# sczhou/CodeFormer

Hardware: NVIDIA H100
Metric: faces_per_sec_512x512_batch32 (higher is better)
Workload: dtype f32 (split-fp16 operands on tensor cores, fp32 accumulate)

## Files before the change

### codeformer_b200/csrc/conv_tc.cu

```cuda

#include <cuda.h>
#include <cuda_fp16.h>
#include <cuda_runtime.h>
#include <stdint.h>

#include <stdlib.h>

#include <atomic>
#include <mutex>

#include "conv_tc.cuh"

namespace cfb {

__global__ void tc_absmax_kernel(const float* __restrict__ w, int64_t total, unsigned* __restrict__ slot) {
  float m = 0.f;
  for (int64_t i = (int64_t)blockIdx.x * blockDim.x + threadIdx.x; i < total; i += (int64_t)gridDim.x * blockDim.x)
    m = fmaxf(m, fabsf(w[i]));
#pragma unroll
  for (int o = 16; o > 0; o >>= 1) m = fmaxf(m, __shfl_xor_sync(0xffffffffu, m, o));
  if ((threadIdx.x & 31) == 0) atomicMax(slot, __float_as_uint(m));
}

__global__ void tc_split_weights_kernel(const float* __restrict__ w, __half* __restrict__ hi, __half* __restrict__ lo,
// ... 282 lines not shown

__device__ __forceinline__ void wg_mma_64x128(float (&d)[64], uint64_t da, uint64_t db, uint32_t accum) {
  asm volatile(
      "{\n\t.reg .pred p;\n\t"
      "setp.ne.b32 p, %66, 0;\n\t"
      "wgmma.mma_async.sync.aligned.m64n128k16.f32.f16.f16 "
      "{%0, %1, %2, %3, %4, %5, %6, %7, %8, %9, %10, %11, %12, %13, %14, %15, "
      "%16, %17, %18, %19, %20, %21, %22, %23, %24, %25, %26, %27, %28, %29, %30, %31, "
      "%32, %33, %34, %35, %36, %37, %38, %39, %40, %41, %42, %43, %44, %45, %46, %47, "
      "%48, %49, %50, %51, %52, %53, %54, %55, %56, %57, %58, %59, %60, %61, %62, %63}, %64, %65, p, 1, 1, 0, 0;\n\t}"
      : "+f"(d[0]), "+f"(d[1]), "+f"(d[2]), "+f"(d[3]), "+f"(d[4]), "+f"(d[5]), "+f"(d[6]), "+f"(d[7]), "+f"(d[8]),
        "+f"(d[9]), "+f"(d[10]), "+f"(d[11]), "+f"(d[12]), "+f"(d[13]), "+f"(d[14]), "+f"(d[15]), "+f"(d[16]),
        "+f"(d[17]), "+f"(d[18]), "+f"(d[19]), "+f"(d[20]), "+f"(d[21]), "+f"(d[22]), "+f"(d[23]), "+f"(d[24]),
        "+f"(d[25]), "+f"(d[26]), "+f"(d[27]), "+f"(d[28]), "+f"(d[29]), "+f"(d[30]), "+f"(d[31]), "+f"(d[32]),
        "+f"(d[33]), "+f"(d[34]), "+f"(d[35]), "+f"(d[36]), "+f"(d[37]), "+f"(d[38]), "+f"(d[39]), "+f"(d[40]),
        "+f"(d[41]), "+f"(d[42]), "+f"(d[43]), "+f"(d[44]), "+f"(d[45]), "+f"(d[46]), "+f"(d[47]), "+f"(d[48]),
        "+f"(d[49]), "+f"(d[50]), "+f"(d[51]), "+f"(d[52]), "+f"(d[53]), "+f"(d[54]), "+f"(d[55]), "+f"(d[56]),
        "+f"(d[57]), "+f"(d[58]), "+f"(d[59]), "+f"(d[60]), "+f"(d[61]), "+f"(d[62]), "+f"(d[63])
      : "l"(da), "l"(db), "r"(accum)
      : "memory");
}
__device__ __forceinline__ void wg_wait_1() { asm volatile("wgmma.wait_group.sync.aligned 1;" ::: "memory"); }

__device__ __forceinline__ bool wg_any(bool v, uint32_t bar_id = 2) {
  uint32_t r;
  asm volatile(
      "{\n\t.reg .pred p, q;\n\t"
      "setp.ne.u32 p, %1, 0;\n\t"
      "bar.red.or.pred q, %2, 128, p;\n\t"
      "selp.u32 %0, 1, 0, q;\n\t}"
      : "=r"(r)
      : "r"((uint32_t)v), "r"(bar_id)
      : "memory");
  return r != 0;
}

__device__ __forceinline__ float ex2_ftz(float x) { float r; asm("ex2.approx.ftz.f32 %0, %1;" : "=f"(r) : "f"(x)); return r; }
__device__ __forceinline__ float rcp_ftz(float x) { float r; asm("rcp.approx.ftz.f32 %0, %1;" : "=f"(r) : "f"(x)); return r; }
__device__ __forceinline__ uint32_t pack_f16x2(float lo, float hi) {
  uint32_t r;
  asm("cvt.rn.f16x2.f32 %0, %1, %2;" : "=r"(r) : "f"(hi), "f"(lo));
  return r;
}
__device__ __forceinline__ float f16_minus_f32(uint32_t h, float c) {
  return __half2float(__ushort_as_half((unsigned short)h)) - c;
}
// ... 23 lines not shown
    float y[2];
#pragma unroll
    for (int e = 0; e < 2; ++e) {
      float v = __uint_as_float(raw[2 * q + e]);
      if (MODE >= 1) v = fmaf(v, sc[2 * q + e], sh[2 * q + e]);
      if (MODE == 2) v = v * rcp_ftz(1.f + ex2_ftz(v * -1.4426950408889634f));
      y[e] = v;
    }
    amax = fmaxf(amax, fmaxf(fabsf(y[0]), fabsf(y[1])));
    hw[q] = pack_f16x2(y[0], y[1]);
    if constexpr (LO) {
      const float d0 = f16_minus_f32(hw[q] & 0xffffu, y[0]);
      const float d1 = f16_minus_f32(hw[q] >> 16, y[1]);
      lw[q] = pack_f16x2(d0, d1) ^ 0x80008000u;
    }
  }
  hv = make_uint4(hw[0], hw[1], hw[2], hw[3]);
  if constexpr (LO) lv = make_uint4(lw[0], lw[1], lw[2], lw[3]);
}
template <int MODE, int RPP, int NPASS, int PW, int ROWS, bool LO = true>
__device__ __forceinline__ void xf_patch(uint32_t src_base, uint32_t hi_base, uint32_t lo_base, int c0, int j, int rsub,
                                         const float (&sc)[8], const float (&sh)[8], bool border, int y0, int x0, int Hin,
                                         int Win, float& amax) {
#pragma unroll
  for (int it = 0; it < NPASS; it += 2) {
    uint4 a[2], b[2];
    bool act[2];
#pragma unroll
    for (int u = 0; u < 2; ++u) {
      const int r = rsub + (it + u) * RPP;
      act[u] = (it + u < NPASS) && (r < ROWS);
      if (act[u]) {
        const uint32_t row = src_base + (uint32_t)r * 128u;
        const uint32_t sw = (row >> 7) & 7u;
        a[u] = lds128(row + (((uint32_t)c0 ^ sw) << 4));
        b[u] = lds128(row + (((uint32_t)(c0 + 1) ^ sw) << 4));
      }
    }
    __syncwarp();
#pragma unroll
    for (int u = 0; u < 2; ++u) {
      if (act[u]) {
        const int r = rsub + (it + u) * RPP;
        uint4 hv, lv;
        xf_chunk<MODE, LO>(a[u], b[u], sc, sh, hv, lv, amax);
        if (border) {
          const int py = r / PW, px = r - py * PW;
// ... 57 lines not shown
  __half* pl_hi;
  __half* pl_lo;
  float* gn_part;
  int gn_cpg;
#if CFB_TC_STAMPS
  long long* dbg;
#endif
};
#if CFB_TC_STAMPS
#define TC_STAMP(i) do { if (p.dbg != nullptr && blockIdx.x == 0) p.dbg[i] = clock64(); } while (0)
#else
#define TC_STAMP(i) do { } while (0)
#endif

constexpr int XF_SKEW = 128;
constexpr int TC_A_BYTES = 128 * 128;

template <int BN>
struct TcCfg {
  static_assert(BN == 64 || BN == 128, "the wgmma engine runs 64- or 128-wide n-tiles");
  static constexpr bool WIDE = BN == 128;
  static constexpr int MMA_WARPS = WIDE ? 8 : 4;
  static constexpr int EPI_WARPS = WIDE ? 4 : 8;
  static constexpr int THREADS = 32 * (MMA_WARPS + 1 + EPI_WARPS);
  static constexpr int B_BYTES = BN * 128;
  static constexpr int STAGE_BYTES = 2 * TC_A_BYTES + 2 * B_BYTES;
  static constexpr int STAGES = 3;
  static constexpr int SLOT_PITCH = BN + 4;
  static constexpr int SLOT_BYTES = 128 * SLOT_PITCH * 4;
  static constexpr int SLOTS = 1;
  static constexpr int STG_BYTES = WIDE ? 0 : 8 * 4096;
  static constexpr int TAIL_BYTES = SLOT_BYTES + 1024  + 512  + STG_BYTES;
  static constexpr int SMEM_BYTES = STAGES * STAGE_BYTES + TAIL_BYTES;
  static constexpr int H_A_PLANE = 23 * 1024;
  static constexpr int H_A_SLOT = 2 * H_A_PLANE;
  static constexpr int H_A_SLOTS = 2;
  static constexpr int H_B_SLOT = 2 * B_BYTES;
  static constexpr int H_B_SLOTS = WIDE ? 2 : 4;
  static constexpr int H_SMEM_BYTES = H_A_SLOTS * H_A_SLOT + H_B_SLOTS * H_B_SLOT + TAIL_BYTES;
  static constexpr int XF_WARPS = WIDE ? 2 : 4;
  static constexpr int XF_THREADS = THREADS + 32 * XF_WARPS + 32;
  static constexpr int X_A_SLOTS = 2;
  static constexpr int X_A_PLANE2 = H_A_PLANE + XF_SKEW;
  static constexpr int X_B_SLOTS = H_B_SLOTS;
  static constexpr int X_SMEM_BYTES = X_A_SLOTS * H_A_SLOT + X_B_SLOTS * H_B_SLOT + TAIL_BYTES;
};

template <int BN, int CPG, bool HALO, bool XF, bool GEN = false, bool K1 = false, bool CM = false, bool SILU = false,
          bool P1 = false>
__global__ void __launch_bounds__(XF ? TcCfg<BN>::XF_THREADS : TcCfg<BN>::THREADS, 1)
conv_tc_kernel(const __grid_constant__ CUtensorMap tmA_hi, const __grid_constant__ CUtensorMap tmA_lo,
               const __grid_constant__ CUtensorMap tmB_hi, const __grid_constant__ CUtensorMap tmB_lo, const TcParams p) {
  static_assert(!XF || HALO, "the fused operand transform exists for the halo engine only");
  static_assert(!GEN || (XF && CPG == 0), "the generalised addressing exists for the fused-transform engine only");
  static_assert(!K1 || (XF && !GEN && CPG == 0), "K1 = fused transform of a 1x1 conv (patch = tile): its own instantiation");
  using Cfg = TcCfg<BN>;
  constexpr bool WIDE = Cfg::WIDE;
  static_assert(!WIDE || (HALO && !GEN && !K1 && CPG != 2), "128-wide tiles exist for the 3x3 / Upsample halo engine");
  static_assert(!CM || (BN == 64 && HALO && !GEN && !K1), "channel-major tiles exist for the 64-channel 3x3 / Upsample halo convs");
  static_assert(!P1 || (!SILU && !K1 && (GEN || WIDE || CM || !HALO)),
                "the single-pass fp16 variant is built for the generalised, 128-wide, channel-major and per-tap engines");
  constexpr int MMA_WARPS = Cfg::MMA_WARPS, EPI_WARPS = Cfg::EPI_WARPS;
  constexpr int A_SLOTS = XF ? Cfg::X_A_SLOTS : Cfg::H_A_SLOTS;
  constexpr int STAGES = Cfg::STAGES;
// ... 29 lines not shown
      mbar_init(smem_u32(afull + a), XF ? Cfg::XF_WARPS : 1);
      mbar_init(smem_u32(aempty + a), MMA_WARPS);
      mbar_init(smem_u32(araw + a), 1);
    }
    asm volatile("prefetch.tensormap [%0];" ::"l"(&tmA_hi) : "memory");
    asm volatile("prefetch.tensormap [%0];" ::"l"(&tmA_lo) : "memory");
    asm volatile("prefetch.tensormap [%0];" ::"l"(&tmB_hi) : "memory");
    asm volatile("prefetch.tensormap [%0];" ::"l"(&tmB_lo) : "memory");
    for (int s = 0; s < NRING; ++s) { mbar_init(smem_u32(full + s), 1); mbar_init(smem_u32(empty + s), MMA_WARPS); }
    for (int a = 0; a < Cfg::SLOTS; ++a) {
      mbar_init(smem_u32(cfull + a), MMA_WARPS);
      mbar_init(smem_u32(cempty + a), EPI_WARPS);
    }
    asm volatile("fence.mbarrier_init.release.cluster;" ::: "memory");
  }
  __syncthreads();
  pdl_launch_dependents();
  pdl_wait();
  if (threadIdx.x == 0) TC_STAMP(1);

  const int total_tiles = p.m_tiles * p.n_tiles;
  const int nk = p.taps * p.kblocks;

  if (warp == 0) {
    {
      int stage = 0;
      uint32_t phase = 0;
      int aslot = 0;
      uint32_t aphase = 0;
      for (int tile = first_tile; tile < total_tiles; tile += tile_step) {
        const int mt = tile / p.n_tiles, nt = tile - mt * p.n_tiles;
        const int mtl = p.up4 ? (mt >> 2) : mt;
        const int par_y = p.up4 ? ((mt & 3) >> 1) : 0, par_x = p.up4 ? (mt & 1) : 0;
        const int per_img = p.tiles_x * p.tiles_y;
        const int n = mtl / per_img;
        const int rem = mtl - n * per_img;
        const int ty = rem / p.tiles_x, tx = rem - ty * p.tiles_x;
        const int y0 = ty * p.BH * p.stride, x0 = tx * p.BW * p.stride;
        if constexpr (HALO) {
          for (int kb = 0; kb < p.kblocks; ++kb) {
            if constexpr (!XF) {
              mbar_wait<500>(smem_u32(aempty + aslot), aphase ^ 1, aborted); if (aborted) goto teardown;
              if (elect_one()) {
                const uint32_t sa = smem_u32(smem + aslot * Cfg::H_A_SLOT);
                const uint32_t ab = smem_u32(afull + aslot);
                mbar_expect_tx(ab, (uint32_t)((P1 ? 1 : 2) * p.PW * p.PH * 128));
// ... 29 lines not shown
              if (elect_one()) {
                if (tile == first_tile && tap == 0 && kb == 0) TC_STAMP(2);
                const uint32_t sa = smem_u32(smem + stage * STAGE_BYTES);
                const int hh = p.heads > 1 ? n % p.heads : 0, nimg = p.heads > 1 ? n / p.heads : n;
                const int a_img = p.a_img_per_head ? n : nimg;
                const int ac = p.a_c0 + hh * p.a_c_head + kb * 64, bc = p.b_c0 + hh * p.b_c_head + kb * 64;
                const int brow = nt * BN + hh * p.b_r_head;
                const int b3 = p.b_batched ? nimg : btap;
                const uint32_t fb = smem_u32(full + stage);
                const bool drop = p.fault && blockIdx.x == 0 && tile == first_tile && kb == 0 && tap == 0;
                mbar_expect_tx(fb, (uint32_t)(P1 ? TC_A_BYTES + Cfg::B_BYTES : Cfg::STAGE_BYTES));
                tma_load_4d(sa, &tmA_hi, fb, ac, x0 + s - p.pad, y0 + r - p.pad, a_img);
                if constexpr (!P1) tma_load_4d(sa + TC_A_BYTES, &tmA_lo, fb, ac, x0 + s - p.pad, y0 + r - p.pad, a_img);
                if (!drop) tma_load_3d(sa + 2 * TC_A_BYTES, &tmB_hi, fb, bc, brow, b3);
                if constexpr (!P1) tma_load_3d(sa + 2 * TC_A_BYTES + Cfg::B_BYTES, &tmB_lo, fb, bc, brow, b3);
              }
              __syncwarp();
              if (++stage == STAGES) { stage = 0; phase ^= 1; }
            }
          }
        }
      }
    }
  } else if (warp == 1) {
    {
      constexpr bool N128 = WIDE || CM;
      constexpr int MH = N128 ? 1 : 2;
      const uint32_t a_sbo = HALO ? (uint32_t)(p.PW * 128) : 1024u;
      const uint32_t a_half = HALO ? (uint32_t)(8 * p.PW * 128) : 8192u;
      const int wq = (int)(threadIdx.x >> 5) & 3;
      const int wg = (int)(threadIdx.x >> 7);
      const uint32_t bar_id = 2u + (uint32_t)wg;
      const uint32_t slot_base = smem_u32(acc_slot);
      int stage = 0;
      uint32_t phase = 0;
      int slot = 0;
      uint32_t slot_phase = 0;
      int aslot = 0;
      uint32_t aphase = 0;
      float acc[MH][N128 ? 64 : 32];
      if constexpr (N128) {
        for (int tile = first_tile; tile < total_tiles; tile += tile_step) {
          const int par = p.up4 ? ((tile / p.n_tiles) & 3) : 0;
          const int par_y = par >> 1, par_x = par & 1;
          for (int c0 = 0; c0 < nk; c0 += p.chunk) {
            const int c1 = min(c0 + p.chunk, nk);
            uint32_t prev_empty = 0, prev_aempty = 0;
            for (int it = c0; it < c1; ++it) {
              const int kb = it / p.taps;
              const int tap = it - kb * p.taps;
              if (tap == 0) {
                mbar_wait(smem_u32(afull + aslot), aphase, aborted);
                if (wg_any(aborted, bar_id)) { wg_wait_all(); aborted = true; goto teardown; }
              }
              int r = (p.taps == 9) ? tap / 3 : 0;
              int sft = (p.taps == 9) ? tap - r * 3 : 0;
              if (p.up4) { r = (tap >> 1) + par_y; sft = (tap & 1) + par_x; }
              const uint32_t a_hi0 = smem_u32(smem + aslot * Cfg::H_A_SLOT) + (uint32_t)((r * p.PW + sft) * 128) +
                                     (uint32_t)wg * a_half;
              const uint32_t a_lo0 = a_hi0 + (uint32_t)(XF ? Cfg::X_A_PLANE2 : Cfg::H_A_PLANE);
              const uint32_t bsm = smem_u32(ring_base + stage * RING_BYTES);
              mbar_wait(smem_u32(full + stage), phase, aborted);
              if (wg_any(aborted, bar_id)) { wg_wait_all(); aborted = true; goto teardown; }
              wg_fence();
#pragma unroll
              for (int k = 0; k < 4; ++k) {
                const uint64_t db_hi = wg_desc(bsm + 32 * k, 1024u), db_lo = wg_desc(bsm + Cfg::B_BYTES + 32 * k, 1024u);
                const uint64_t da_hi = wg_desc(a_hi0 + 32 * k, a_sbo), da_lo = wg_desc(a_lo0 + 32 * k, a_sbo);
                if constexpr (P1 && CM) {
                  wg_mma_64x128(acc[0], db_hi, da_hi, (it == c0 && k == 0) ? 0u : 1u);
                } else if constexpr (P1) {
                  wg_mma_64x128(acc[0], da_hi, db_hi, (it == c0 && k == 0) ? 0u : 1u);
                } else if constexpr (CM) {
                  wg_mma_64x128(acc[0], db_hi, da_lo, (it == c0 && k == 0) ? 0u : 1u);
                  wg_mma_64x128(acc[0], db_lo, da_hi, 1u);
                  wg_mma_64x128(acc[0], db_hi, da_hi, 1u);
                } else {
                  wg_mma_64x128(acc[0], da_lo, db_hi, (it == c0 && k == 0) ? 0u : 1u);
                  wg_mma_64x128(acc[0], da_hi, db_lo, 1u);
                  wg_mma_64x128(acc[0], da_hi, db_hi, 1u);
                }
              }
              wg_commit();
              wg_wait_1();
              __syncwarp();
              mbar_arrive_if(prev_empty, lane == 0 && prev_empty != 0);
              mbar_arrive_if(prev_aempty, lane == 0 && prev_aempty != 0);
              prev_empty = smem_u32(empty + stage);
              prev_aempty = tap == p.taps - 1 ? smem_u32(aempty + aslot) : 0u;
              if (++stage == NRING) { stage = 0; phase ^= 1; }
              if (tap == p.taps - 1 && ++aslot == A_SLOTS) { aslot = 0; aphase ^= 1; }
            }
            wg_wait_all();
            __syncwarp();
            mbar_arrive_if(prev_empty, lane == 0);
            mbar_arrive_if(prev_aempty, lane == 0 && prev_aempty != 0);
            if constexpr (CM) {
              mbar_wait(smem_u32(cempty + slot), slot_phase ^ 1, aborted);
              if (wg_any(aborted, bar_id)) { aborted = true; goto teardown; }
              const uint32_t st0 = slot_base + (uint32_t)(slot * Cfg::SLOT_BYTES) +
                                   (uint32_t)((2 * (lane & 3) * Cfg::SLOT_PITCH + wq * 16 + (lane >> 2)) * 4);
#pragma unroll
              for (int j = 0; j < 16; ++j) {
#pragma unroll
                for (int h8 = 0; h8 < 2; ++h8) {
#pragma unroll
                  for (int e = 0; e < 2; ++e) {
                    const uint32_t a = st0 + (uint32_t)(((8 * j + e) * Cfg::SLOT_PITCH + 8 * h8) * 4);
                    asm volatile("st.shared.f32 [%0], %1;" ::"r"(a), "f"(acc[0][4 * j + 2 * h8 + e]) : "memory");
                  }
                }
              }
              __syncwarp();
              if (lane == 0) mbar_arrive(smem_u32(cfull + slot));
              if (++slot == Cfg::SLOTS) { slot = 0; slot_phase ^= 1; }
              continue;
            }
            const bool first_chunk = c0 == 0;
            if (first_chunk) {
              mbar_wait(smem_u32(cempty + slot), slot_phase ^ 1, aborted);
              if (wg_any(aborted, bar_id)) { aborted = true; goto teardown; }
            }
            const uint32_t sbase = slot_base + (uint32_t)(slot * Cfg::SLOT_BYTES);
            const int row = wg * 64 + wq * 16 + (lane >> 2);
#pragma unroll
            for (int j = 0; j < 16; ++j) {
#pragma unroll
              for (int h8 = 0; h8 < 2; ++h8) {
                const uint32_t e = sbase + (uint32_t)(((row + 8 * h8) * Cfg::SLOT_PITCH + 8 * j + 2 * (lane & 3)) * 4);
                float x = 0.f, y = 0.f;
                if (!first_chunk) asm volatile("ld.shared.v2.f32 {%0, %1}, [%2];" : "=f"(x), "=f"(y) : "r"(e) : "memory");
                x = __fadd_rn(x, acc[0][4 * j + 2 * h8]);
                y = __fadd_rn(y, acc[0][4 * j + 2 * h8 + 1]);
                asm volatile("st.shared.v2.f32 [%0], {%1, %2};" ::"r"(e), "f"(x), "f"(y) : "memory");
              }
            }
          }
          if constexpr (!CM) {
            __syncwarp();
            if (lane == 0) mbar_arrive(smem_u32(cfull + slot));
            if (++slot == Cfg::SLOTS) { slot = 0; slot_phase ^= 1; }
          }
        }
      } else {
      for (int tile = first_tile; tile < total_tiles; tile += tile_step) {
        const int par = p.up4 ? ((tile / p.n_tiles) & 3) : 0;
        const int par_y = par >> 1, par_x = par & 1;
        for (int it = 0; it < nk; ++it) {
          uint32_t a_hi0, a_lo0, bsm;
          int tap = 0;
          if constexpr (HALO) {
            const int kb = it / p.taps;
            tap = it - kb * p.taps;
            if (tap == 0) { mbar_wait(smem_u32(afull + aslot), aphase, aborted); if (wg_any(aborted)) { aborted = true; goto teardown; } }
            int r = (p.taps == 9) ? tap / 3 : 0;
            int sft = (p.taps == 9) ? tap - r * 3 : 0;
            if (p.up4) { r = (tap >> 1) + par_y; sft = (tap & 1) + par_x; }
            const uint32_t aoff = (uint32_t)((r * p.PW + sft) * 128);
            a_hi0 = smem_u32(smem + aslot * Cfg::H_A_SLOT) + aoff;
            a_lo0 = a_hi0 + (uint32_t)(XF ? Cfg::X_A_PLANE2 : Cfg::H_A_PLANE);
            bsm = smem_u32(ring_base + stage * RING_BYTES);
          } else {
            a_hi0 = smem_u32(smem + stage * STAGE_BYTES);
            a_lo0 = a_hi0 + TC_A_BYTES;
            bsm = a_hi0 + 2 * TC_A_BYTES;
          }
          mbar_wait(smem_u32(full + stage), phase, aborted); if (wg_any(aborted)) { aborted = true; goto teardown; }
          if (blockIdx.x == 0 && threadIdx.x == 0 && tile == first_tile && it == 0) TC_STAMP(3);
          const uint32_t first = (it % p.chunk) == 0 ? 1u : 0u;
          wg_fence();
#pragma unroll
          for (int k = 0; k < 4; ++k) {
            const uint64_t db_hi = wg_desc(bsm + 32 * k, 1024u), db_lo = wg_desc(bsm + Cfg::B_BYTES + 32 * k, 1024u);
#pragma unroll
            for (int mh = 0; mh < 2; ++mh) {
              const uint64_t da_hi = wg_desc(a_hi0 + mh * a_half + 32 * k, a_sbo), da_lo = wg_desc(a_lo0 + mh * a_half + 32 * k, a_sbo);
              if constexpr (P1) {
                wg_mma_64x64(acc[mh], da_hi, db_hi, (first && k == 0) ? 0u : 1u);
              } else {
                wg_mma_64x64(acc[mh], da_lo, db_hi, (first && k == 0) ? 0u : 1u);
                wg_mma_64x64(acc[mh], da_hi, db_lo, 1u);
                wg_mma_64x64(acc[mh], da_hi, db_hi, 1u);
              }
            }
          }
          wg_commit();
          wg_wait_all();
          __syncwarp();
          if (lane == 0) mbar_arrive(smem_u32(empty + stage));
          if (++stage == NRING) { stage = 0; phase ^= 1; }
          if constexpr (HALO) {
            if (tap == p.taps - 1) {
              if (lane == 0) mbar_arrive(smem_u32(aempty + aslot));
              if (++aslot == A_SLOTS) { aslot = 0; aphase ^= 1; }
            }
          }
          if ((it % p.chunk) == p.chunk - 1 || it == nk - 1) {
            mbar_wait(smem_u32(cempty + slot), slot_phase ^ 1, aborted); if (wg_any(aborted)) { aborted = true; goto teardown; }
            const uint32_t sbase = slot_base + (uint32_t)(slot * Cfg::SLOT_BYTES);
#pragma unroll
            for (int mh = 0; mh < 2; ++mh) {
              const int row = mh * 64 + wq * 16 + (lane >> 2);
#pragma unroll
              for (int j = 0; j < 8; ++j) {
                const uint32_t e = sbase + (uint32_t)((row * Cfg::SLOT_PITCH + 8 * j + 2 * (lane & 3)) * 4);
                asm volatile("st.shared.v2.f32 [%0], {%1, %2};" ::"r"(e), "f"(acc[mh][4 * j]), "f"(acc[mh][4 * j + 1]) : "memory");
                asm volatile("st.shared.v2.f32 [%0], {%1, %2};" ::"r"(e + 8 * Cfg::SLOT_PITCH * 4), "f"(acc[mh][4 * j + 2]),
                             "f"(acc[mh][4 * j + 3]) : "memory");
              }
            }
            __syncwarp();
            if (lane == 0) mbar_arrive(smem_u32(cfull + slot));
            if (++slot == Cfg::SLOTS) { slot = 0; slot_phase ^= 1; }
          }
        }
      }
      }
    }
  } else if (XF && warp == 2 + EPI_WARPS + Cfg::XF_WARPS) {
    if constexpr (XF) {
      int aslot = 0;
      uint32_t aphase = 0;
      for (int tile = first_tile; tile < total_tiles; tile += tile_step) {
        const int mt0 = tile / p.n_tiles;
        const int mt = p.up4 ? (mt0 >> 2) : mt0;
        const int per_img = p.tiles_x * p.tiles_y;
        const int n = mt / per_img;
        const int rem = mt - n * per_img;
        const int ty = rem / p.tiles_x, tx = rem - ty * p.tiles_x;
        const int y0 = ty * p.BH, x0 = tx * p.BW;
        for (int kb = 0; kb < p.kblocks; ++kb) {
          mbar_wait<500>(smem_u32(aempty + aslot), aphase ^ 1, aborted); if (aborted) goto teardown;
          if (elect_one()) {
            const uint32_t sa = smem_u32(smem + aslot * Cfg::H_A_SLOT);
            const uint32_t rb = smem_u32(araw + aslot);
            const bool src0 = kb < p.a_split;
            const CUtensorMap* src = src0 ? &tmA_hi : &tmA_lo;
            const int c0 = (src0 ? kb : kb - p.a_split) * 64;
            if (tile == first_tile && kb == 0) TC_STAMP(10);
            mbar_expect_tx(rb, (uint32_t)(2 * p.PW * p.PH * 128));
            tma_load_4d(sa, src, rb, c0, x0 - p.pad, y0 - p.pad, n);
// ... 77 lines not shown
                const uint32_t hs = base0 + (uint32_t)rs * 128u, hd = base0 + (uint32_t)r * 128u;
                const uint32_t ls = lo_base + (uint32_t)rs * 128u, ld = lo_base + (uint32_t)r * 128u;
                const uint4 hv = lds128(hs + ((((uint32_t)j) ^ ((hs >> 7) & 7u)) << 4));
                if constexpr (P1) {
                  sts128(hd + ((((uint32_t)j) ^ ((hd >> 7) & 7u)) << 4), hv);
                } else {
                  const uint4 lv = lds128(ls + ((((uint32_t)j) ^ ((ls >> 7) & 7u)) << 4));
                  sts128(hd + ((((uint32_t)j) ^ ((hd >> 7) & 7u)) << 4), hv);
                  sts128(ld + ((((uint32_t)j) ^ ((ld >> 7) & 7u)) << 4), lv);
                }
              }
            }
          }
          asm volatile("fence.proxy.async.shared::cta;" ::: "memory");
          __syncwarp();
          if (lane == 0) mbar_arrive(smem_u32(afull + aslot));
          if (t == 0 && tile == first_tile && kb == 0) TC_STAMP(12);
          if (t == 0 && tile == first_tile + tile_step && kb == 0) TC_STAMP(20);
          if (++aslot == A_SLOTS) { aslot = 0; aphase ^= 1; }
        }
      }
      if (amax > 65504.f) report_overflow();
    }
  } else {
    constexpr int HC = BN * 4 / EPI_WARPS;
    const int lg = (warp - 2) & 3;
    const int half = (warp - 2) >> 2;
    const int row = lg * 32 + lane;
    const int cbase = half * HC;
    const float wsi = __ldg(p.wscale_inv);
    const int BW = HALO ? 8 : p.BW, BH = HALO ? 16 : p.BH;
    const int bw_shift = HALO ? 3 : ((BW & (BW - 1)) == 0 ? __ffs(BW) - 1 : -1);
    const int64_t SW = (int64_t)(p.up4 ? 2 : 1) * (HALO ? p.Cout : p.out_pitch), SH = SW * p.Wo;
    const int ts = p.up4 ? 2 : 1;
    const bool whole_tiles = HALO || (p.tiles_y * BH * ts == p.Ho && p.tiles_x * BW * ts == p.Wo);
    int slot = 0;
    uint32_t slot_phase = 0;
    float omax = 0.f;
    for (int tile = first_tile; tile < total_tiles; tile += tile_step) {
      const int pm = tile / p.n_tiles, nt = tile - pm * p.n_tiles;
      const int mt = pm;
      const int mtl = p.up4 ? (mt >> 2) : mt;
      const int per_img = p.tiles_x * p.tiles_y;
      const int nb = mtl / per_img;
      const int rem = mtl - nb * per_img;
      const bool hsplit = !HALO && p.heads > 1 && !p.out_per_head;
// ... 198 lines not shown
          constexpr int CL = (CPG >= 4) ? CPG / 4 : 1;
          if (rsub == 0 && (cch & (CL - 1)) == 0) {
            float* gp = p.gn_part + ((int64_t)mt * 4 + lg) * 64;
            if constexpr (CPG == 2) {
              *reinterpret_cast<float4*>(gp + (colq / 2) * 2) = make_float4(s0, q0, s1, q1);
            } else {
              *reinterpret_cast<float2*>(gp + (colq / CPG) * 2) = make_float2(s0, q0);
            }
          }
        }
        __syncwarp();
      }
      }
      if constexpr (WIDE) {
        if (lane == 0) mbar_arrive(smem_u32(cempty + slot));
        if (++slot == Cfg::SLOTS) { slot = 0; slot_phase ^= 1; }
      }
      if (warp == 2 && lane == 0 && tile == first_tile) TC_STAMP(16);
      if (warp == 2 && lane == 0 && tile == first_tile + tile_step) TC_STAMP(18);
    }
    if (omax > 65504.f) report_overflow();
    if (warp == 2 && lane == 0) TC_STAMP(13);
  }

teardown:
  if (aborted) {
    const long long t0 = clock64();
    while (clock64() - t0 < 400000) {}
  }
  __syncthreads();
  if (threadIdx.x == 0) TC_STAMP(8);
}

int tc_bind_status_word(unsigned* host_mapped_dev_ptr, long long wait_limit_cycles) {
  const unsigned zero = 0;
  CFB_CUDA(cudaMemcpyToSymbol(g_status_host, &host_mapped_dev_ptr, sizeof(host_mapped_dev_ptr)));
  CFB_CUDA(cudaMemcpyToSymbol(g_wait_limit, &wait_limit_cycles, sizeof(wait_limit_cycles)));
  CFB_CUDA(cudaMemcpyToSymbol(g_abort, &zero, sizeof(zero)));
  return 0;
}
static std::atomic<int> g_inject_fault{0};
static std::atomic<long long*> g_stamps{nullptr};
int tc_set_stamps(long long* dev_ptr) { g_stamps.store(dev_ptr); return 0; }
int tc_inject_fault(int kind) { g_inject_fault.store(kind); return 0; }
int tc_clear_abort() {
  const unsigned zero = 0;
// ... 119 lines not shown
  CFB_CUDA(cudaGetDevice(&dev));
  const uint64_t bit = 1ull << (dev & 63);
  if (!(attr_done.load(std::memory_order_acquire) & bit)) {
    CFB_CUDA(cudaFuncSetAttribute(conv_tc_kernel<BN, CPG, HALO, XF, GEN, K1, CM, SILU, P1>, cudaFuncAttributeMaxDynamicSharedMemorySize, SMEM));
    attr_done.fetch_or(bit, std::memory_order_release);
  }
  const int total = p.m_tiles * p.n_tiles;
  const int grid = total < sm_count ? total : sm_count;
  CFB_LAUNCH_PDL((conv_tc_kernel<BN, CPG, HALO, XF, GEN, K1, CM, SILU, P1>), dim3((unsigned)grid), dim3(THREADS), (size_t)SMEM, st,
                 m.a_hi, m.a_lo, m.b_hi, m.b_lo, p);
  return 0;
}
template <int CPG>
static int launch_tc_p1(const TcMaps& m, const TcParams& p, int sm_count, cudaStream_t st, bool gen, int tile) {
  constexpr bool T = true, F = false;
  const bool halo3 = p.PW == 10 && p.PH == 18;
  if (p.out_act != OUT_SILU) {
    if (gen) {
      if constexpr (CPG == 0) {
        if (p.xform && halo3) return launch_tc2<64, 0, T, T, T, F, F, F, T>(m, p, sm_count, st);
      }
    } else if (tile == 128 && halo3) {
      if constexpr (CPG == 4 || CPG == 8 || CPG == 16) {
        if (p.xform) return launch_tc2<128, CPG, T, T, F, F, F, F, T>(m, p, sm_count, st);
      }
      if constexpr (CPG != 2) {
        if (!p.xform) return launch_tc2<128, CPG, T, F, F, F, F, F, T>(m, p, sm_count, st);
      }
    } else if (tile == TC_TILE_CM && halo3) {
      if constexpr (CPG == 2) {
        if (p.xform) return launch_tc2<64, 2, T, T, F, F, T, F, T>(m, p, sm_count, st);
      }
      if constexpr (CPG <= 2) {
        if (!p.xform) return launch_tc2<64, CPG, T, F, F, F, T, F, T>(m, p, sm_count, st);
      }
    } else if (tile == TC_TILE_N && !p.xform && p.PW == 0 && p.taps == 1) {
      if constexpr (CPG == 0) return launch_tc2<64, 0, F, F, F, F, F, F, T>(m, p, sm_count, st);
    }
  }
  CFB_REQUIRE(false, "conv_tc: single-pass fp16 is built for the generalised engine, the 128-wide and channel-major halo tiles "
                     "and the per-tap 1x1 conv, without the SiLU epilogue");
  return 1;
}

template <int CPG>
static int launch_tc(const TcMaps& m, const TcParams& p, int sm_count, cudaStream_t st, bool gen = false, int tile = TC_TILE_N,
                     bool single_pass = false) {
  CFB_REQUIRE(p.out_act != OUT_SILU || (CPG == 0 && (gen || (!p.xform && p.PW == 0))),
              "conv_tc: the SiLU epilogue is built for the per-tap and generalised engines without statistics");
  if (single_pass) return launch_tc_p1<CPG>(m, p, sm_count, st, gen, tile);
  if (tile == TC_TILE_CM) {
    if constexpr (CPG <= 2) {
      CFB_REQUIRE(p.PW == 10 && p.PH == 18, "conv_tc: channel-major tiles need the 3x3 / Upsample halo engine");
      if (p.xform) return launch_tc2<64, CPG, true, true, false, false, true>(m, p, sm_count, st);
      return launch_tc2<64, CPG, true, false, false, false, true>(m, p, sm_count, st);
    } else {
      CFB_REQUIRE(false, "conv_tc: channel-major tiles need Cout % 128 == 64");
    }
  }
  if (tile == 128) {
    if constexpr (CPG != 2) {
      CFB_REQUIRE(p.PW == 10 && p.PH == 18, "conv_tc: 128-wide tiles need the 3x3 / Upsample halo engine");
      if (p.xform) return launch_tc2<128, CPG, true, true>(m, p, sm_count, st);
      return launch_tc2<128, CPG, true>(m, p, sm_count, st);
    } else {
      CFB_REQUIRE(false, "conv_tc: 128-wide tiles need Cout % 128 == 0");
    }
  }
  if constexpr (CPG == 0) {
    if (gen) {
      CFB_REQUIRE(p.xform && p.PW == 10 && p.PH == 18, "conv_tc: generalised variant needs the halo + transform engine");
      if (p.out_act == OUT_SILU) return launch_tc2<64, 0, true, true, true, false, false, true>(m, p, sm_count, st);
      return launch_tc2<64, 0, true, true, true>(m, p, sm_count, st);
    }
    if (p.out_act == OUT_SILU) return launch_tc2<64, 0, false, false, false, false, false, true>(m, p, sm_count, st);
  }
  if (p.xform) {
    CFB_REQUIRE((p.PW == 10 && p.PH == 18) || (p.PW == 8 && p.PH == 16 && p.taps == 1),
                "conv_tc: fused operand transform needs the halo engine");
    if (p.taps == 1) {
      if constexpr (CPG == 0) return launch_tc2<64, 0, true, true, false, true>(m, p, sm_count, st);
      else { CFB_REQUIRE(false, "conv_tc: the 1x1 fused transform is built without statistics"); }
    }
    return launch_tc2<64, CPG, true, true>(m, p, sm_count, st);
  }
  if (p.PW > 0) return launch_tc2<64, CPG, true>(m, p, sm_count, st);
// ... 570 lines not shown
```

Baseline: 173.9.

## Split registers with setmaxnreg and keep cross-chunk accumulator in registers for wide tiles

For the 128-wide halo conv tiles, the block is padded to four warpgroups so setmaxnreg can lower registers for the producer, epilogue and transform warps and raise them for the MMA warpgroups. The MMA role moves into a shared include. In the wide path, partial sums across k-chunks are now kept in a 64-entry register array and written to the shared slot once per tile, instead of a load-add-store on the slot after every chunk. The wide fused-transform path now hardcodes 9 taps without up4 and guards this at launch. The costs are extra idle threads and more register pressure, and the xf_patch unroll is capped for large NPASS.

```diff
diff --git a/codeformer_b200/csrc/conv_tc.cu b/codeformer_b200/csrc/conv_tc.cu
--- a/codeformer_b200/csrc/conv_tc.cu
+++ b/codeformer_b200/csrc/conv_tc.cu
@@ -328,6 +328,14 @@
 }
 __device__ __forceinline__ void wg_wait_1() { asm volatile("wgmma.wait_group.sync.aligned 1;" ::: "memory"); }
 
+template <int PITCH, int J = 0>
+__device__ __forceinline__ void wide_slot_store(uint32_t base, const float (&v)[64]) {
+  asm volatile("st.shared.v2.f32 [%0+%5], {%1, %2};\n\tst.shared.v2.f32 [%0+%6], {%3, %4};"
+               ::"r"(base), "f"(v[4 * J]), "f"(v[4 * J + 1]), "f"(v[4 * J + 2]), "f"(v[4 * J + 3]), "n"(32 * J),
+                 "n"(32 * J + 32 * PITCH) : "memory");
+  if constexpr (J + 1 < 16) wide_slot_store<PITCH, J + 1>(base, v);
+}
+
 __device__ __forceinline__ bool wg_any(bool v, uint32_t bar_id = 2) {
   uint32_t r;
   asm volatile(
@@ -397,7 +405,7 @@
 __device__ __forceinline__ void xf_patch(uint32_t src_base, uint32_t hi_base, uint32_t lo_base, int c0, int j, int rsub,
                                          const float (&sc)[8], const float (&sh)[8], bool border, int y0, int x0, int Hin,
                                          int Win, float& amax) {
-#pragma unroll
+#pragma unroll (NPASS > 16 ? 1 : NPASS)
   for (int it = 0; it < NPASS; it += 2) {
     uint4 a[2], b[2];
     bool act[2];
@@ -501,7 +509,9 @@
   static constexpr bool WIDE = BN == 128;
   static constexpr int MMA_WARPS = WIDE ? 8 : 4;
   static constexpr int EPI_WARPS = WIDE ? 4 : 8;
-  static constexpr int THREADS = 32 * (MMA_WARPS + 1 + EPI_WARPS);
+  static constexpr int XF_WARPS = WIDE ? 2 : 4;
+  static constexpr int THREADS = WIDE ? 32 * (MMA_WARPS + 1 + EPI_WARPS + XF_WARPS + 1) : 32 * (MMA_WARPS + 1 + EPI_WARPS);
+  static constexpr int MMA_REGS = 160, HELPER_REGS = 256 - MMA_REGS;
   static constexpr int B_BYTES = BN * 128;
   static constexpr int STAGE_BYTES = 2 * TC_A_BYTES + 2 * B_BYTES;
   static constexpr int STAGES = 3;
@@ -517,8 +527,7 @@
   static constexpr int H_B_SLOT = 2 * B_BYTES;
   static constexpr int H_B_SLOTS = WIDE ? 2 : 4;
   static constexpr int H_SMEM_BYTES = H_A_SLOTS * H_A_SLOT + H_B_SLOTS * H_B_SLOT + TAIL_BYTES;
-  static constexpr int XF_WARPS = WIDE ? 2 : 4;
-  static constexpr int XF_THREADS = THREADS + 32 * XF_WARPS + 32;
+  static constexpr int XF_THREADS = 32 * (MMA_WARPS + 1 + EPI_WARPS + XF_WARPS + 1);
   static constexpr int X_A_SLOTS = 2;
   static constexpr int X_A_PLANE2 = H_A_PLANE + XF_SKEW;
   static constexpr int X_B_SLOTS = H_B_SLOTS;
@@ -594,6 +603,10 @@
   const int total_tiles = p.m_tiles * p.n_tiles;
   const int nk = p.taps * p.kblocks;
 
+  static_assert(!WIDE || (Cfg::THREADS == 512 && Cfg::XF_THREADS == 512 && Cfg::MMA_WARPS == 8),
+                "the setmaxnreg split needs 2 MMA + 2 helper warpgroups");
+  if (!WIDE || warp != 1) {
+  if constexpr (WIDE) asm volatile("setmaxnreg.dec.sync.aligned.u32 %0;" ::"n"(Cfg::HELPER_REGS) : "memory");
   if (warp == 0) {
     {
       int stage = 0;
@@ -669,201 +682,8 @@
         }
       }
     }
-  } else if (warp == 1) {
-    {
-      constexpr bool N128 = WIDE || CM;
-      constexpr int MH = N128 ? 1 : 2;
-      const uint32_t a_sbo = HALO ? (uint32_t)(p.PW * 128) : 1024u;
-      const uint32_t a_half = HALO ? (uint32_t)(8 * p.PW * 128) : 8192u;
-      const int wq = (int)(threadIdx.x >> 5) & 3;
-      const int wg = (int)(threadIdx.x >> 7);
-      const uint32_t bar_id = 2u + (uint32_t)wg;
-      const uint32_t slot_base = smem_u32(acc_slot);
-      int stage = 0;
-      uint32_t phase = 0;
-      int slot = 0;
-      uint32_t slot_phase = 0;
-      int aslot = 0;
-      uint32_t aphase = 0;
-      float acc[MH][N128 ? 64 : 32];
-      if constexpr (N128) {
-        for (int tile = first_tile; tile < total_tiles; tile += tile_step) {
-          const int par = p.up4 ? ((tile / p.n_tiles) & 3) : 0;
-          const int par_y = par >> 1, par_x = par & 1;
-          for (int c0 = 0; c0 < nk; c0 += p.chunk) {
-            const int c1 = min(c0 + p.chunk, nk);
-            uint32_t prev_empty = 0, prev_aempty = 0;
-            for (int it = c0; it < c1; ++it) {
-              const int kb = it / p.taps;
-              const int tap = it - kb * p.taps;
-              if (tap == 0) {
-                mbar_wait(smem_u32(afull + aslot), aphase, aborted);
-                if (wg_any(aborted, bar_id)) { wg_wait_all(); aborted = true; goto teardown; }
-              }
-              int r = (p.taps == 9) ? tap / 3 : 0;
-              int sft = (p.taps == 9) ? tap - r * 3 : 0;
-              if (p.up4) { r = (tap >> 1) + par_y; sft = (tap & 1) + par_x; }
-              const uint32_t a_hi0 = smem_u32(smem + aslot * Cfg::H_A_SLOT) + (uint32_t)((r * p.PW + sft) * 128) +
-                                     (uint32_t)wg * a_half;
-              const uint32_t a_lo0 = a_hi0 + (uint32_t)(XF ? Cfg::X_A_PLANE2 : Cfg::H_A_PLANE);
-              const uint32_t bsm = smem_u32(ring_base + stage * RING_BYTES);
-              mbar_wait(smem_u32(full + stage), phase, aborted);
-              if (wg_any(aborted, bar_id)) { wg_wait_all(); aborted = true; goto teardown; }
-              wg_fence();
-#pragma unroll
-              for (int k = 0; k < 4; ++k) {
-                const uint64_t db_hi = wg_desc(bsm + 32 * k, 1024u), db_lo = wg_desc(bsm + Cfg::B_BYTES + 32 * k, 1024u);
-                const uint64_t da_hi = wg_desc(a_hi0 + 32 * k, a_sbo), da_lo = wg_desc(a_lo0 + 32 * k, a_sbo);
-                if constexpr (P1 && CM) {
-                  wg_mma_64x128(acc[0], db_hi, da_hi, (it == c0 && k == 0) ? 0u : 1u);
-                } else if constexpr (P1) {
-                  wg_mma_64x128(acc[0], da_hi, db_hi, (it == c0 && k == 0) ? 0u : 1u);
-                } else if constexpr (CM) {
-                  wg_mma_64x128(acc[0], db_hi, da_lo, (it == c0 && k == 0) ? 0u : 1u);
-                  wg_mma_64x128(acc[0], db_lo, da_hi, 1u);
-                  wg_mma_64x128(acc[0], db_hi, da_hi, 1u);
-                } else {
-                  wg_mma_64x128(acc[0], da_lo, db_hi, (it == c0 && k == 0) ? 0u : 1u);
-                  wg_mma_64x128(acc[0], da_hi, db_lo, 1u);
-                  wg_mma_64x128(acc[0], da_hi, db_hi, 1u);
-                }
-              }
-              wg_commit();
-              wg_wait_1();
-              __syncwarp();
-              mbar_arrive_if(prev_empty, lane == 0 && prev_empty != 0);
-              mbar_arrive_if(prev_aempty, lane == 0 && prev_aempty != 0);
-              prev_empty = smem_u32(empty + stage);
-              prev_aempty = tap == p.taps - 1 ? smem_u32(aempty + aslot) : 0u;
-              if (++stage == NRING) { stage = 0; phase ^= 1; }
-              if (tap == p.taps - 1 && ++aslot == A_SLOTS) { aslot = 0; aphase ^= 1; }
-            }
-            wg_wait_all();
-            __syncwarp();
-            mbar_arrive_if(prev_empty, lane == 0);
-            mbar_arrive_if(prev_aempty, lane == 0 && prev_aempty != 0);
-            if constexpr (CM) {
-              mbar_wait(smem_u32(cempty + slot), slot_phase ^ 1, aborted);
-              if (wg_any(aborted, bar_id)) { aborted = true; goto teardown; }
-              const uint32_t st0 = slot_base + (uint32_t)(slot * Cfg::SLOT_BYTES) +
-                                   (uint32_t)((2 * (lane & 3) * Cfg::SLOT_PITCH + wq * 16 + (lane >> 2)) * 4);
-#pragma unroll
-              for (int j = 0; j < 16; ++j) {
-#pragma unroll
-                for (int h8 = 0; h8 < 2; ++h8) {
-#pragma unroll
-                  for (int e = 0; e < 2; ++e) {
-                    const uint32_t a = st0 + (uint32_t)(((8 * j + e) * Cfg::SLOT_PITCH + 8 * h8) * 4);
-                    asm volatile("st.shared.f32 [%0], %1;" ::"r"(a), "f"(acc[0][4 * j + 2 * h8 + e]) : "memory");
-                  }
-                }
-              }
-              __syncwarp();
-              if (lane == 0) mbar_arrive(smem_u32(cfull + slot));
-              if (++slot == Cfg::SLOTS) { slot = 0; slot_phase ^= 1; }
-              continue;
-            }
-            const bool first_chunk = c0 == 0;
-            if (first_chunk) {
-              mbar_wait(smem_u32(cempty + slot), slot_phase ^ 1, aborted);
-              if (wg_any(aborted, bar_id)) { aborted = true; goto teardown; }
-            }
-            const uint32_t sbase = slot_base + (uint32_t)(slot * Cfg::SLOT_BYTES);
-            const int row = wg * 64 + wq * 16 + (lane >> 2);
-#pragma unroll
-            for (int j = 0; j < 16; ++j) {
-#pragma unroll
-              for (int h8 = 0; h8 < 2; ++h8) {
-                const uint32_t e = sbase + (uint32_t)(((row + 8 * h8) * Cfg::SLOT_PITCH + 8 * j + 2 * (lane & 3)) * 4);
-                float x = 0.f, y = 0.f;
-                if (!first_chunk) asm volatile("ld.shared.v2.f32 {%0, %1}, [%2];" : "=f"(x), "=f"(y) : "r"(e) : "memory");
-                x = __fadd_rn(x, acc[0][4 * j + 2 * h8]);
-                y = __fadd_rn(y, acc[0][4 * j + 2 * h8 + 1]);
-                asm volatile("st.shared.v2.f32 [%0], {%1, %2};" ::"r"(e), "f"(x), "f"(y) : "memory");
-              }
-            }
-          }
-          if constexpr (!CM) {
-            __syncwarp();
-            if (lane == 0) mbar_arrive(smem_u32(cfull + slot));
-            if (++slot == Cfg::SLOTS) { slot = 0; slot_phase ^= 1; }
-          }
-        }
-      } else {
-      for (int tile = first_tile; tile < total_tiles; tile += tile_step) {
-        const int par = p.up4 ? ((tile / p.n_tiles) & 3) : 0;
-        const int par_y = par >> 1, par_x = par & 1;
-        for (int it = 0; it < nk; ++it) {
-          uint32_t a_hi0, a_lo0, bsm;
-          int tap = 0;
-          if constexpr (HALO) {
-            const int kb = it / p.taps;
-            tap = it - kb * p.taps;
-            if (tap == 0) { mbar_wait(smem_u32(afull + aslot), aphase, aborted); if (wg_any(aborted)) { aborted = true; goto teardown; } }
-            int r = (p.taps == 9) ? tap / 3 : 0;
-            int sft = (p.taps == 9) ? tap - r * 3 : 0;
-            if (p.up4) { r = (tap >> 1) + par_y; sft = (tap & 1) + par_x; }
-            const uint32_t aoff = (uint32_t)((r * p.PW + sft) * 128);
-            a_hi0 = smem_u32(smem + aslot * Cfg::H_A_SLOT) + aoff;
-            a_lo0 = a_hi0 + (uint32_t)(XF ? Cfg::X_A_PLANE2 : Cfg::H_A_PLANE);
-            bsm = smem_u32(ring_base + stage * RING_BYTES);
-          } else {
-            a_hi0 = smem_u32(smem + stage * STAGE_BYTES);
-            a_lo0 = a_hi0 + TC_A_BYTES;
-            bsm = a_hi0 + 2 * TC_A_BYTES;
-          }
-          mbar_wait(smem_u32(full + stage), phase, aborted); if (wg_any(aborted)) { aborted = true; goto teardown; }
-          if (blockIdx.x == 0 && threadIdx.x == 0 && tile == first_tile && it == 0) TC_STAMP(3);
-          const uint32_t first = (it % p.chunk) == 0 ? 1u : 0u;
-          wg_fence();
-#pragma unroll
-          for (int k = 0; k < 4; ++k) {
-            const uint64_t db_hi = wg_desc(bsm + 32 * k, 1024u), db_lo = wg_desc(bsm + Cfg::B_BYTES + 32 * k, 1024u);
-#pragma unroll
-            for (int mh = 0; mh < 2; ++mh) {
-              const uint64_t da_hi = wg_desc(a_hi0 + mh * a_half + 32 * k, a_sbo), da_lo = wg_desc(a_lo0 + mh * a_half + 32 * k, a_sbo);
-              if constexpr (P1) {
-                wg_mma_64x64(acc[mh], da_hi, db_hi, (first && k == 0) ? 0u : 1u);
-              } else {
-                wg_mma_64x64(acc[mh], da_lo, db_hi, (first && k == 0) ? 0u : 1u);
-                wg_mma_64x64(acc[mh], da_hi, db_lo, 1u);
-                wg_mma_64x64(acc[mh], da_hi, db_hi, 1u);
-              }
-            }
-          }
-          wg_commit();
-          wg_wait_all();
-          __syncwarp();
-          if (lane == 0) mbar_arrive(smem_u32(empty + stage));
-          if (++stage == NRING) { stage = 0; phase ^= 1; }
-          if constexpr (HALO) {
-            if (tap == p.taps - 1) {
-              if (lane == 0) mbar_arrive(smem_u32(aempty + aslot));
-              if (++aslot == A_SLOTS) { aslot = 0; aphase ^= 1; }
-            }
-          }
-          if ((it % p.chunk) == p.chunk - 1 || it == nk - 1) {
-            mbar_wait(smem_u32(cempty + slot), slot_phase ^ 1, aborted); if (wg_any(aborted)) { aborted = true; goto teardown; }
-            const uint32_t sbase = slot_base + (uint32_t)(slot * Cfg::SLOT_BYTES);
-#pragma unroll
-            for (int mh = 0; mh < 2; ++mh) {
-              const int row = mh * 64 + wq * 16 + (lane >> 2);
-#pragma unroll
-              for (int j = 0; j < 8; ++j) {
-                const uint32_t e = sbase + (uint32_t)((row * Cfg::SLOT_PITCH + 8 * j + 2 * (lane & 3)) * 4);
-                asm volatile("st.shared.v2.f32 [%0], {%1, %2};" ::"r"(e), "f"(acc[mh][4 * j]), "f"(acc[mh][4 * j + 1]) : "memory");
-                asm volatile("st.shared.v2.f32 [%0], {%1, %2};" ::"r"(e + 8 * Cfg::SLOT_PITCH * 4), "f"(acc[mh][4 * j + 2]),
-                             "f"(acc[mh][4 * j + 3]) : "memory");
-              }
-            }
-            __syncwarp();
-            if (lane == 0) mbar_arrive(smem_u32(cfull + slot));
-            if (++slot == Cfg::SLOTS) { slot = 0; slot_phase ^= 1; }
-          }
-        }
-      }
-      }
-    }
+  } else if (!WIDE && warp == 1) {
+#include "conv_tc_mma_role.cuh"
   } else if (XF && warp == 2 + EPI_WARPS + Cfg::XF_WARPS) {
     if constexpr (XF) {
       int aslot = 0;
@@ -987,6 +807,7 @@
       }
       if (amax > 65504.f) report_overflow();
     }
+  } else if (WIDE && !XF && warp >= 2 + EPI_WARPS) {
   } else {
     constexpr int HC = BN * 4 / EPI_WARPS;
     const int lg = (warp - 2) & 3;
@@ -1231,6 +1052,10 @@
     if (omax > 65504.f) report_overflow();
     if (warp == 2 && lane == 0) TC_STAMP(13);
   }
+  } else {
+    if constexpr (WIDE) asm volatile("setmaxnreg.inc.sync.aligned.u32 %0;" ::"n"(Cfg::MMA_REGS) : "memory");
+#include "conv_tc_mma_role.cuh"
+  }
 
 teardown:
   if (aborted) {
@@ -1396,6 +1221,7 @@
       }
     } else if (tile == 128 && halo3) {
       if constexpr (CPG == 4 || CPG == 8 || CPG == 16) {
+        CFB_REQUIRE(!p.xform || (p.taps == 9 && !p.up4), "conv_tc: 128-wide fused-transform tiles are built for 3x3 'same' convs");
         if (p.xform) return launch_tc2<128, CPG, T, T, F, F, F, F, T>(m, p, sm_count, st);
       }
       if constexpr (CPG != 2) {
@@ -1435,7 +1261,10 @@
   if (tile == 128) {
     if constexpr (CPG != 2) {
       CFB_REQUIRE(p.PW == 10 && p.PH == 18, "conv_tc: 128-wide tiles need the 3x3 / Upsample halo engine");
-      if (p.xform) return launch_tc2<128, CPG, true, true>(m, p, sm_count, st);
+      if (p.xform) {
+        CFB_REQUIRE(p.taps == 9 && !p.up4, "conv_tc: 128-wide fused-transform tiles are built for 3x3 'same' convs");
+        return launch_tc2<128, CPG, true, true>(m, p, sm_count, st);
+      }
       return launch_tc2<128, CPG, true>(m, p, sm_count, st);
     } else {
       CFB_REQUIRE(false, "conv_tc: 128-wide tiles need Cout % 128 == 0");
diff --git a/codeformer_b200/csrc/conv_tc_mma_role.cuh b/codeformer_b200/csrc/conv_tc_mma_role.cuh
--- /dev/null
+++ b/codeformer_b200/csrc/conv_tc_mma_role.cuh
@@ -0,0 +1,192 @@
+    {
+      constexpr bool N128 = WIDE || CM;
+      constexpr int MH = N128 ? 1 : 2;
+      const uint32_t a_sbo = HALO ? (uint32_t)(p.PW * 128) : 1024u;
+      const uint32_t a_half = HALO ? (uint32_t)(8 * p.PW * 128) : 8192u;
+      const int wq = (int)(threadIdx.x >> 5) & 3;
+      const int wg = (int)(threadIdx.x >> 7);
+      const uint32_t bar_id = 2u + (uint32_t)wg;
+      const uint32_t slot_base = smem_u32(acc_slot);
+      int stage = 0;
+      uint32_t phase = 0;
+      int slot = 0;
+      uint32_t slot_phase = 0;
+      int aslot = 0;
+      uint32_t aphase = 0;
+      float acc[MH][N128 ? 64 : 32];
+      float run[WIDE ? 64 : 1];
+      if constexpr (N128) {
+        const int taps = (WIDE && XF) ? 9 : p.taps;
+        const bool up4 = !(WIDE && XF) && p.up4;
+        for (int tile = first_tile; tile < total_tiles; tile += tile_step) {
+          const int par = up4 ? ((tile / p.n_tiles) & 3) : 0;
+          const int par_y = par >> 1, par_x = par & 1;
+          for (int c0 = 0; c0 < nk; c0 += p.chunk) {
+            const int c1 = min(c0 + p.chunk, nk);
+            uint32_t prev_empty = 0, prev_aempty = 0;
+            for (int it = c0; it < c1; ++it) {
+              const int kb = it / taps;
+              const int tap = it - kb * taps;
+              if (tap == 0) {
+                mbar_wait(smem_u32(afull + aslot), aphase, aborted);
+                if (wg_any(aborted, bar_id)) { wg_wait_all(); aborted = true; goto teardown; }
+              }
+              int r = (taps == 9) ? tap / 3 : 0;
+              int sft = (taps == 9) ? tap - r * 3 : 0;
+              if (up4) { r = (tap >> 1) + par_y; sft = (tap & 1) + par_x; }
+              const uint32_t a_hi0 = smem_u32(smem + aslot * Cfg::H_A_SLOT) + (uint32_t)((r * p.PW + sft) * 128) +
+                                     (uint32_t)wg * a_half;
+              const uint32_t a_lo0 = a_hi0 + (uint32_t)(XF ? Cfg::X_A_PLANE2 : Cfg::H_A_PLANE);
+              const uint32_t bsm = smem_u32(ring_base + stage * RING_BYTES);
+              mbar_wait(smem_u32(full + stage), phase, aborted);
+              if (wg_any(aborted, bar_id)) { wg_wait_all(); aborted = true; goto teardown; }
+              wg_fence();
+#pragma unroll
+              for (int k = 0; k < 4; ++k) {
+                const uint64_t db_hi = wg_desc(bsm + 32 * k, 1024u), db_lo = wg_desc(bsm + Cfg::B_BYTES + 32 * k, 1024u);
+                const uint64_t da_hi = wg_desc(a_hi0 + 32 * k, a_sbo), da_lo = wg_desc(a_lo0 + 32 * k, a_sbo);
+                if constexpr (P1 && CM) {
+                  wg_mma_64x128(acc[0], db_hi, da_hi, (it == c0 && k == 0) ? 0u : 1u);
+                } else if constexpr (P1) {
+                  wg_mma_64x128(acc[0], da_hi, db_hi, (it == c0 && k == 0) ? 0u : 1u);
+                } else if constexpr (CM) {
+                  wg_mma_64x128(acc[0], db_hi, da_lo, (it == c0 && k == 0) ? 0u : 1u);
+                  wg_mma_64x128(acc[0], db_lo, da_hi, 1u);
+                  wg_mma_64x128(acc[0], db_hi, da_hi, 1u);
+                } else {
+                  wg_mma_64x128(acc[0], da_lo, db_hi, (it == c0 && k == 0) ? 0u : 1u);
+                  wg_mma_64x128(acc[0], da_hi, db_lo, 1u);
+                  wg_mma_64x128(acc[0], da_hi, db_hi, 1u);
+                }
+              }
+              wg_commit();
+              wg_wait_1();
+              __syncwarp();
+              mbar_arrive_if(prev_empty, lane == 0 && prev_empty != 0);
+              mbar_arrive_if(prev_aempty, lane == 0 && prev_aempty != 0);
+              prev_empty = smem_u32(empty + stage);
+              prev_aempty = tap == taps - 1 ? smem_u32(aempty + aslot) : 0u;
+              if (++stage == NRING) { stage = 0; phase ^= 1; }
+              if (tap == taps - 1 && ++aslot == A_SLOTS) { aslot = 0; aphase ^= 1; }
+            }
+            wg_wait_all();
+            __syncwarp();
+            mbar_arrive_if(prev_empty, lane == 0);
+            mbar_arrive_if(prev_aempty, lane == 0 && prev_aempty != 0);
+            if constexpr (CM) {
+              mbar_wait(smem_u32(cempty + slot), slot_phase ^ 1, aborted);
+              if (wg_any(aborted, bar_id)) { aborted = true; goto teardown; }
+              const uint32_t st0 = slot_base + (uint32_t)(slot * Cfg::SLOT_BYTES) +
+                                   (uint32_t)((2 * (lane & 3) * Cfg::SLOT_PITCH + wq * 16 + (lane >> 2)) * 4);
+#pragma unroll
+              for (int j = 0; j < 16; ++j) {
+#pragma unroll
+                for (int h8 = 0; h8 < 2; ++h8) {
+#pragma unroll
+                  for (int e = 0; e < 2; ++e) {
+                    const uint32_t a = st0 + (uint32_t)(((8 * j + e) * Cfg::SLOT_PITCH + 8 * h8) * 4);
+                    asm volatile("st.shared.f32 [%0], %1;" ::"r"(a), "f"(acc[0][4 * j + 2 * h8 + e]) : "memory");
+                  }
+                }
+              }
+              __syncwarp();
+              if (lane == 0) mbar_arrive(smem_u32(cfull + slot));
+              if (++slot == Cfg::SLOTS) { slot = 0; slot_phase ^= 1; }
+              continue;
+            }
+            if constexpr (WIDE) {
+              if (c0 == 0) {
+#pragma unroll
+                for (int i = 0; i < 64; ++i) run[i] = __fadd_rn(0.f, acc[0][i]);
+              } else {
+#pragma unroll
+                for (int i = 0; i < 64; ++i) run[i] = __fadd_rn(run[i], acc[0][i]);
+              }
+            }
+          }
+          if constexpr (!CM) {
+            mbar_wait(smem_u32(cempty + slot), slot_phase ^ 1, aborted);
+            if (wg_any(aborted, bar_id)) { aborted = true; goto teardown; }
+            const int row = wg * 64 + wq * 16 + (lane >> 2);
+            wide_slot_store<Cfg::SLOT_PITCH>(slot_base + (uint32_t)(slot * Cfg::SLOT_BYTES) +
+                                                 (uint32_t)((row * Cfg::SLOT_PITCH + 2 * (lane & 3)) * 4), run);
+            __syncwarp();
+            if (lane == 0) mbar_arrive(smem_u32(cfull + slot));
+            if (++slot == Cfg::SLOTS) { slot = 0; slot_phase ^= 1; }
+          }
+        }
+      } else {
+      for (int tile = first_tile; tile < total_tiles; tile += tile_step) {
+        const int par = p.up4 ? ((tile / p.n_tiles) & 3) : 0;
+        const int par_y = par >> 1, par_x = par & 1;
+        for (int it = 0; it < nk; ++it) {
+          uint32_t a_hi0, a_lo0, bsm;
+          int tap = 0;
+          if constexpr (HALO) {
+            const int kb = it / p.taps;
+            tap = it - kb * p.taps;
+            if (tap == 0) { mbar_wait(smem_u32(afull + aslot), aphase, aborted); if (wg_any(aborted)) { aborted = true; goto teardown; } }
+            int r = (p.taps == 9) ? tap / 3 : 0;
+            int sft = (p.taps == 9) ? tap - r * 3 : 0;
+            if (p.up4) { r = (tap >> 1) + par_y; sft = (tap & 1) + par_x; }
+            const uint32_t aoff = (uint32_t)((r * p.PW + sft) * 128);
+            a_hi0 = smem_u32(smem + aslot * Cfg::H_A_SLOT) + aoff;
+            a_lo0 = a_hi0 + (uint32_t)(XF ? Cfg::X_A_PLANE2 : Cfg::H_A_PLANE);
+            bsm = smem_u32(ring_base + stage * RING_BYTES);
+          } else {
+            a_hi0 = smem_u32(smem + stage * STAGE_BYTES);
+            a_lo0 = a_hi0 + TC_A_BYTES;
+            bsm = a_hi0 + 2 * TC_A_BYTES;
+          }
+          mbar_wait(smem_u32(full + stage), phase, aborted); if (wg_any(aborted)) { aborted = true; goto teardown; }
+          if (blockIdx.x == 0 && threadIdx.x == 0 && tile == first_tile && it == 0) TC_STAMP(3);
+          const uint32_t first = (it % p.chunk) == 0 ? 1u : 0u;
+          wg_fence();
+#pragma unroll
+          for (int k = 0; k < 4; ++k) {
+            const uint64_t db_hi = wg_desc(bsm + 32 * k, 1024u), db_lo = wg_desc(bsm + Cfg::B_BYTES + 32 * k, 1024u);
+#pragma unroll
+            for (int mh = 0; mh < 2; ++mh) {
+              const uint64_t da_hi = wg_desc(a_hi0 + mh * a_half + 32 * k, a_sbo), da_lo = wg_desc(a_lo0 + mh * a_half + 32 * k, a_sbo);
+              if constexpr (P1) {
+                wg_mma_64x64(acc[mh], da_hi, db_hi, (first && k == 0) ? 0u : 1u);
+              } else {
+                wg_mma_64x64(acc[mh], da_lo, db_hi, (first && k == 0) ? 0u : 1u);
+                wg_mma_64x64(acc[mh], da_hi, db_lo, 1u);
+                wg_mma_64x64(acc[mh], da_hi, db_hi, 1u);
+              }
+            }
+          }
+          wg_commit();
+          wg_wait_all();
+          __syncwarp();
+          if (lane == 0) mbar_arrive(smem_u32(empty + stage));
+          if (++stage == NRING) { stage = 0; phase ^= 1; }
+          if constexpr (HALO) {
+            if (tap == p.taps - 1) {
+              if (lane == 0) mbar_arrive(smem_u32(aempty + aslot));
+              if (++aslot == A_SLOTS) { aslot = 0; aphase ^= 1; }
+            }
+          }
+          if ((it % p.chunk) == p.chunk - 1 || it == nk - 1) {
+            mbar_wait(smem_u32(cempty + slot), slot_phase ^ 1, aborted); if (wg_any(aborted)) { aborted = true; goto teardown; }
+            const uint32_t sbase = slot_base + (uint32_t)(slot * Cfg::SLOT_BYTES);
+#pragma unroll
+            for (int mh = 0; mh < 2; ++mh) {
+              const int row = mh * 64 + wq * 16 + (lane >> 2);
+#pragma unroll
+              for (int j = 0; j < 8; ++j) {
+                const uint32_t e = sbase + (uint32_t)((row * Cfg::SLOT_PITCH + 8 * j + 2 * (lane & 3)) * 4);
+                asm volatile("st.shared.v2.f32 [%0], {%1, %2};" ::"r"(e), "f"(acc[mh][4 * j]), "f"(acc[mh][4 * j + 1]) : "memory");
+                asm volatile("st.shared.v2.f32 [%0], {%1, %2};" ::"r"(e + 8 * Cfg::SLOT_PITCH * 4), "f"(acc[mh][4 * j + 2]),
+                             "f"(acc[mh][4 * j + 3]) : "memory");
+              }
+            }
+            __syncwarp();
+            if (lane == 0) mbar_arrive(smem_u32(cfull + slot));
+            if (++slot == Cfg::SLOTS) { slot = 0; slot_phase ^= 1; }
+          }
+        }
+      }
+      }
+    }
```

Result: faster. 187.5 (median of 6 runs) (+7.8%).
